# lbcb-sci/raven

Measured on NVIDIA H100. Metric: overlaps/s, higher is better.
Workload: dtype u64

## Files before the change

### raven_b200/csrc/map.cu

```cuda
#include <algorithm>

#include "engine.cuh"
#include "seed.cuh"

namespace rvn {

namespace {

constexpr int kThreads = 256;

__global__ void __launch_bounds__(kThreads)
ProbeKernel(IndexView ix, ValView q_val,
            const uint64_t* __restrict__ q_org, uint64_t q_begin, uint64_t n_q,
            bool avoid_equal, bool avoid_symmetric,
            uint32_t* __restrict__ cnt, uint32_t* __restrict__ first,
            uint8_t* __restrict__ filt) {
  const uint64_t i = static_cast<uint64_t>(blockIdx.x) * kThreads + threadIdx.x;
  if (i >= n_q) return;
  const uint32_t lhs_id = static_cast<uint32_t>(q_org[q_begin + i] >> 32);
  ProbeRun(ix, q_val[q_begin + i], lhs_id, avoid_equal, avoid_symmetric, first + i, cnt + i,
           filt + i);
}

struct HitStore {
// ... 431 lines not shown
      const uint64_t* Pb = P + jb;
      const IdxT* idx = MINI + jb + b;
      const bool strand = G[jb] & 1;
      for (uint32_t kk = 1, l = 0; kk <= longest; ++kk) {
        const uint32_t prev = static_cast<uint32_t>(Pb[idx[kk - 1]] >> 32);
        const uint32_t cur =
            kk < longest ? static_cast<uint32_t>(Pb[idx[kk]] >> 32) : 0xFFFFFFFFu;
        if (cur - prev > cp.gap) {
          if (kk - l >= cp.chain) {
            uint32_t lm = 0, lb_ = 0, le = 0, rm = 0, rb_ = 0, re = 0;
            for (uint32_t m = l; m < kk; ++m) {
              const uint64_t pp = Pb[idx[m]];
              const uint32_t lp = static_cast<uint32_t>(pp >> 32);
              if (lp > le) {
                lm += le - lb_;
                lb_ = lp;
              }
              le = lp + cp.k;
              uint32_t rp = static_cast<uint32_t>(pp);
              rp = strand ? rp : (1U << 31) - (rp + cp.k - 1);
              if (rp > re) {
                rm += re - rb_;
                rb_ = rp;
              }
              re = rp + cp.k;
            }
            lm += le - lb_;
            rm += re - rb_;
            if (min(lm, rm) >= cp.matches) ++emitted;
          }
          l = kk;
        }
      }
    }
    wk.CNT[b] = emitted;
    wk.IE[b] = static_cast<IdxT>(longest);
  }
  __syncthreads();

  uint32_t carry = 0;
  __shared__ uint32_t sh_total;
  {
    uint32_t local = 0;
    for (uint32_t b = threadIdx.x; b < nb; b += THREADS) local += wk.CNT[b];
    uint32_t tot;
    BlockExclusiveSum<uint32_t, THREADS>(local, sm32, &tot);
    if (threadIdx.x == 0) {
      sh_total = tot;
      sh_base = tot ? atomicAdd(ovl_counter, static_cast<unsigned long long>(tot))
                    : 0ULL;
    }
    __syncthreads();
  }
  const uint32_t total = sh_total;
  const uint64_t base = sh_base;
  *out_base = base;
  if (total == 0 || base + total > ovl_cap) return total;

  for (uint32_t b0 = 0; b0 < nb; b0 += THREADS) {
    const uint32_t b = b0 + threadIdx.x;
    const uint32_t mine = b < nb ? wk.CNT[b] : 0;
    uint32_t tot;
    const uint32_t ex = BlockExclusiveSum<uint32_t, THREADS>(mine, sm32, &tot);
    if (mine) {
      rvn_overlap* dst = ovl_raw + base + carry + ex;
      uint64_t* kdst = ovl_key ? ovl_key + base + carry + ex : nullptr;
      uint32_t seq = carry + ex;
      const uint32_t jb = wk.IB[b];
      const uint32_t longest = wk.IE[b];
      const uint64_t* Pb = P + jb;
      const IdxT* idx = MINI + jb + b;
      const bool strand = G[jb] & 1;
      const uint32_t rhs_id = static_cast<uint32_t>(G[jb] & 0xFFFFFFFFu) >> 1;
      for (uint32_t kk = 1, l = 0; kk <= longest; ++kk) {
        const uint32_t prev = static_cast<uint32_t>(Pb[idx[kk - 1]] >> 32);
        const uint32_t cur =
            kk < longest ? static_cast<uint32_t>(Pb[idx[kk]] >> 32) : 0xFFFFFFFFu;
        if (cur - prev > cp.gap) {
          if (kk - l >= cp.chain) {
            uint32_t lm = 0, lb_ = 0, le = 0, rm = 0, rb_ = 0, re = 0;
            for (uint32_t m = l; m < kk; ++m) {
              const uint64_t pp = Pb[idx[m]];
              const uint32_t lp = static_cast<uint32_t>(pp >> 32);
              if (lp > le) {
                lm += le - lb_;
                lb_ = lp;
              }
              le = lp + cp.k;
              uint32_t rp = static_cast<uint32_t>(pp);
              rp = strand ? rp : (1U << 31) - (rp + cp.k - 1);
              if (rp > re) {
                rm += re - rb_;
                rb_ = rp;
              }
              re = rp + cp.k;
            }
            lm += le - lb_;
            rm += re - rb_;
            if (min(lm, rm) >= cp.matches) {
              const uint64_t pf = Pb[idx[l]], pl = Pb[idx[kk - 1]];
              rvn_overlap o;
              o.lhs_id = lhs_id;
              o.lhs_begin = static_cast<uint32_t>(pf >> 32);
              o.lhs_end = cp.k + static_cast<uint32_t>(pl >> 32);
              o.rhs_id = rhs_id;
              o.rhs_begin = strand ? static_cast<uint32_t>(pf)
                                   : static_cast<uint32_t>(pl);
              o.rhs_end = cp.k + (strand ? static_cast<uint32_t>(pl)
                                         : static_cast<uint32_t>(pf));
              o.score = min(lm, rm);
              o.strand = strand;
              *dst++ = o;
              if (kdst) *kdst++ = key_hi | seq++;
            }
          }
          l = kk;
        }
      }
    }
    carry += tot;
  }
  return total;
}

constexpr uint32_t kChainSmemCap = 65535;
constexpr uint32_t kSplitMaxTable = 8192;
constexpr uint32_t kPairMaxHits = 8191;
constexpr uint32_t kThreadPairMax = 48;

struct GroupDesc {
  uint32_t hit_off, cnt, gid, lhs_id;
};

struct SplitLayout {
  uint32_t hs, gpad;
  size_t hk, hc, gl, bytes;
};

__host__ __device__ inline SplitLayout MakeSplitLayout(uint32_t n) {
  SplitLayout L;
  uint32_t hs = 64;
  while (hs < n + 1 && hs < kSplitMaxTable) hs <<= 1;
  L.hs = hs;
  uint32_t gpad = 2;
  while (gpad < n / 4 + 1 && gpad < hs) gpad <<= 1;
  L.gpad = gpad;
  size_t o = 0;
  L.hk = o; o += 4ULL * hs;
  L.hc = o; o += 4ULL * hs;
  L.gl = o; o += 8ULL * gpad;
  L.bytes = (o + 15) & ~size_t(15);
  return L;
}

__device__ __forceinline__ uint32_t HashGid(uint32_t x) {
  x ^= x >> 16;
  x *= 0x7feb352dU;
  x ^= x >> 15;
  x *= 0x846ca68bU;
  x ^= x >> 16;
  return x;
}

template <int THREADS, int MINB>
__global__ void __launch_bounds__(THREADS, MINB)
SplitKernel(const uint64_t* __restrict__ h_grp, const uint64_t* __restrict__ h_pos,
            const uint64_t* __restrict__ read_hit_off,
            const uint32_t* __restrict__ lhs_ids,
            const uint32_t* __restrict__ read_list,
            unsigned long long* __restrict__ totals,
            GroupDesc* __restrict__ desc, uint32_t* __restrict__ desc_cnt,
            uint32_t* __restrict__ desc_idx, uint32_t* __restrict__ g_diag,
            uint64_t* __restrict__ g_pos, uint64_t* __restrict__ group_loc,
            uint32_t* __restrict__ fallback_list,
            unsigned int* __restrict__ fallback_cnt) {
  extern __shared__ __align__(16) unsigned char smem[];
  __shared__ uint32_t sm32[34];
  __shared__ uint32_t sh_bail;
  __shared__ unsigned long long sh_gbase, sh_hbase;
  const uint32_t r = read_list[blockIdx.x];
  const uint64_t hb = read_hit_off[r];
  const uint32_t n = static_cast<uint32_t>(read_hit_off[r + 1] - hb);
  const SplitLayout L = MakeSplitLayout(n);
  uint32_t* HK = reinterpret_cast<uint32_t*>(smem + L.hk);
  uint32_t* HC = reinterpret_cast<uint32_t*>(smem + L.hc);
  uint64_t* GL = reinterpret_cast<uint64_t*>(smem + L.gl);
  const uint32_t hmask = L.hs - 1;
  const uint64_t* hg = h_grp + hb;
  const uint64_t* hp = h_pos + hb;

  for (uint32_t i = threadIdx.x; i < L.hs; i += THREADS) {
    HK[i] = 0xFFFFFFFFu;
    HC[i] = 0;
  }
  if (threadIdx.x == 0) sh_bail = 0;
  __syncthreads();
  for (uint32_t i = threadIdx.x; i < n; i += THREADS) {
    const uint32_t gid = static_cast<uint32_t>(hg[i] >> 32);
    uint32_t s = HashGid(gid) & hmask;
    uint32_t probes = 0;
    while (true) {
      const uint32_t prev = atomicCAS(&HK[s], 0xFFFFFFFFu, gid);
      if (prev == 0xFFFFFFFFu || prev == gid) break;
      s = (s + 1) & hmask;
      if (++probes > hmask) {
        sh_bail = 1;
        break;
      }
    }
    if (probes <= hmask) atomicAdd(&HC[s], 1u);
  }
  __syncthreads();
  if (sh_bail) {
    if (threadIdx.x == 0) fallback_list[atomicAdd(fallback_cnt, 1u)] = r;
    return;
  }

  uint32_t carry = 0;
  for (uint32_t b = 0; b < L.hs; b += THREADS) {
    const uint32_t s = b + threadIdx.x;
    const uint32_t cnt = s < L.hs ? HC[s] : 0;
    const uint32_t keep = cnt >= 4;
    if (cnt > kPairMaxHits) sh_bail = 1;
    uint32_t tot;
    const uint32_t ex = BlockExclusiveSum<uint32_t, THREADS>(
        keep ? ((cnt << 16) | 1u) : 0u, sm32, &tot);
    if (s < L.hs) {
      if (keep) {
        const uint32_t at = carry + ex;
        GL[at & 0xFFFF] = (static_cast<uint64_t>(HK[s]) << 32) | s;
        HC[s] = (cnt << 16) | (at >> 16);
      } else {
        HC[s] = 0xFFFFFFFFu;
      }
    }
    carry += tot;
  }
  const uint32_t ng = carry & 0xFFFF, nh = carry >> 16;
  __syncthreads();
  if (sh_bail) {
    if (threadIdx.x == 0) fallback_list[atomicAdd(fallback_cnt, 1u)] = r;
    return;
  }
  if (ng == 0) {
    if (threadIdx.x == 0) group_loc[r] = 0;
    return;
  }

  uint32_t gpad = 2;
  while (gpad < ng) gpad <<= 1;
  for (uint32_t i = ng + threadIdx.x; i < gpad; i += THREADS) GL[i] = ~0ULL;
  if (threadIdx.x == 0) {
    sh_gbase = atomicAdd(&totals[0], static_cast<unsigned long long>(ng));
    sh_hbase = atomicAdd(&totals[1], static_cast<unsigned long long>(nh));
  }
  __syncthreads();
  for (uint32_t size = 2; size <= gpad; size <<= 1) {
    for (uint32_t stride = size >> 1; stride > 0; stride >>= 1) {
      for (uint32_t t = threadIdx.x; t < (gpad >> 1); t += THREADS) {
        const uint32_t i = 2 * t - (t & (stride - 1));
        const uint32_t j = i + stride;
        const uint64_t a = GL[i], c2 = GL[j];
        if ((a > c2) == ((i & size) == 0)) {
          GL[i] = c2;
          GL[j] = a;
        }
      }
      __syncthreads();
    }
  }
  const uint64_t gbase = sh_gbase, hbase = sh_hbase;
  const uint32_t lhs_id = lhs_ids[r];
  for (uint32_t q = threadIdx.x; q < ng; q += THREADS) {
    const uint64_t e = GL[q];
    const uint32_t s = static_cast<uint32_t>(e);
    const uint32_t v = HC[s];
    GroupDesc d;
    d.hit_off = static_cast<uint32_t>(hbase) + (v & 0xFFFF);
    d.cnt = v >> 16;
    d.gid = static_cast<uint32_t>(e >> 32);
    d.lhs_id = lhs_id;
    desc[gbase + q] = d;
    desc_cnt[gbase + q] = d.cnt;
    desc_idx[gbase + q] = static_cast<uint32_t>(gbase + q);
    HC[s] = v & 0xFFFF;
  }
  if (threadIdx.x == 0) group_loc[r] = (gbase << 24) | ng;
  __syncthreads();

  for (uint32_t i = threadIdx.x; i < n; i += THREADS) {
    const uint64_t g = hg[i];
    const uint32_t gid = static_cast<uint32_t>(g >> 32);
    uint32_t s = HashGid(gid) & hmask;
    while (HK[s] != gid) s = (s + 1) & hmask;
    if (HC[s] == 0xFFFFFFFFu) continue;
    const uint64_t at = hbase + atomicAdd(&HC[s], 1u);
    g_diag[at] = static_cast<uint32_t>(g);
    g_pos[at] = hp[i];
  }
}

struct Column {
  uint64_t* P;
  uint32_t* D;
  uint32_t T;
  __device__ __forceinline__ uint64_t& p(uint32_t i) const { return P[i * T]; }
  __device__ __forceinline__ uint32_t& d(uint32_t i) const { return D[i * T]; }
};

__device__ __forceinline__ void BandChain(const Column& c, uint32_t jb, uint32_t ie,
                                          bool strand, uint32_t lhs_id,
                                          uint32_t rhs_id, const ChainParams& cp,
                                          uint64_t key_hi, uint32_t* seq,
                                          rvn_overlap* __restrict__ out,
                                          uint64_t* __restrict__ out_key,
                                          unsigned long long* __restrict__ out_cnt,
                                          uint64_t out_cap) {
  const uint32_t len = ie - jb;
  if (len < cp.chain) return;
  for (uint32_t a = 1; a < len; ++a) {
    const uint64_t pv = c.p(jb + a);
    if (c.p(jb + a - 1) <= pv) continue;
    uint32_t lo = 0, hi = a - 1;
    while (lo < hi) {
      const uint32_t mid = (lo + hi) >> 1;
      if (c.p(jb + mid) > pv) {
        hi = mid;
      } else {
        lo = mid + 1;
      }
    }
    for (uint32_t b = a; b > lo; --b) c.p(jb + b) = c.p(jb + b - 1);
    c.p(jb + lo) = pv;
  }
  auto mini_get = [&](uint32_t x) -> uint32_t { return c.d(jb + x) & 0xFFFFu; };
  auto mini_set = [&](uint32_t x, uint32_t v) {
    c.d(jb + x) = (c.d(jb + x) & 0xFFFF0000u) | v;
  };
  auto pred_get = [&](uint32_t x) -> uint32_t { return c.d(jb + x) >> 16; };
  auto pred_set = [&](uint32_t x, uint32_t v) {
    c.d(jb + x) = (c.d(jb + x) & 0xFFFFu) | (v << 16);
  };
  uint32_t longest = 0;
  for (uint32_t t = 0; t < len; ++t) {
    const uint64_t cur = c.p(jb + t);
    const uint32_t cl = static_cast<uint32_t>(cur >> 32);
    const uint32_t cr = static_cast<uint32_t>(cur);
    uint32_t lo = 1, hi = longest;
    while (lo <= hi) {
      const uint32_t mid = lo + (hi - lo) / 2;
      const uint64_t tail = c.p(jb + mini_get(mid - 1));
      const uint32_t tl = static_cast<uint32_t>(tail >> 32);
      const uint32_t tr = static_cast<uint32_t>(tail);
      if (tl < cl && (strand ? tr < cr : tr > cr)) {
        lo = mid + 1;
      } else {
        hi = mid - 1;
      }
    }
    pred_set(t, lo > 1 ? mini_get(lo - 2) : 0u);
    mini_set(lo - 1, t);
    longest = max(longest, lo);
  }
  if (longest < cp.chain) return;
  {
    uint32_t j = mini_get(longest - 1);
    for (uint32_t i = 0; i < longest; ++i) {
      const uint32_t pj = pred_get(j);
      mini_set(longest - 1 - i, j);
      j = pj;
    }
  }
  for (uint32_t kk = 1, l = 0; kk <= longest; ++kk) {
    const uint32_t prev = static_cast<uint32_t>(c.p(jb + mini_get(kk - 1)) >> 32);
    const uint32_t cur = kk < longest
                             ? static_cast<uint32_t>(c.p(jb + mini_get(kk)) >> 32)
                             : 0xFFFFFFFFu;
    if (cur - prev > cp.gap) {
      if (kk - l >= cp.chain) {
        uint32_t lm = 0, lb_ = 0, le = 0, rm = 0, rb_ = 0, re = 0;
        for (uint32_t m = l; m < kk; ++m) {
          const uint64_t pp = c.p(jb + mini_get(m));
          const uint32_t lp = static_cast<uint32_t>(pp >> 32);
          if (lp > le) {
            lm += le - lb_;
            lb_ = lp;
          }
          le = lp + cp.k;
          uint32_t rp = static_cast<uint32_t>(pp);
          rp = strand ? rp : (1U << 31) - (rp + cp.k - 1);
          if (rp > re) {
            rm += re - rb_;
            rb_ = rp;
          }
          re = rp + cp.k;
        }
        lm += le - lb_;
        rm += re - rb_;
        if (min(lm, rm) >= cp.matches) {
          const uint64_t pf = c.p(jb + mini_get(l)), pl = c.p(jb + mini_get(kk - 1));
          rvn_overlap o;
          o.lhs_id = lhs_id;
          o.lhs_begin = static_cast<uint32_t>(pf >> 32);
          o.lhs_end = cp.k + static_cast<uint32_t>(pl >> 32);
          o.rhs_id = rhs_id;
          o.rhs_begin = strand ? static_cast<uint32_t>(pf) : static_cast<uint32_t>(pl);
          o.rhs_end = cp.k + (strand ? static_cast<uint32_t>(pl)
                                     : static_cast<uint32_t>(pf));
          o.score = min(lm, rm);
          o.strand = strand;
          const unsigned long long slot = atomicAdd(out_cnt, 1ULL);
          if (slot < out_cap) {
            out[slot] = o;
            out_key[slot] = key_hi | (*seq)++;
          }
        }
      }
      l = kk;
    }
  }
}

__global__ void GroupChainKernel(const GroupDesc* __restrict__ desc,
                                 const uint32_t* __restrict__ order, uint64_t first,
                                 uint64_t last, uint32_t m_cap,
                                 const uint32_t* __restrict__ g_diag,
                                 const uint64_t* __restrict__ g_pos, ChainParams cp,
                                 rvn_overlap* __restrict__ out,
                                 uint64_t* __restrict__ out_key,
                                 unsigned long long* __restrict__ out_cnt,
                                 uint64_t out_cap) {
  extern __shared__ __align__(16) unsigned char smem[];
  const uint32_t T = blockDim.x;
  const uint64_t t = first + static_cast<uint64_t>(blockIdx.x) * T + threadIdx.x;
  if (t >= last) return;
  Column c;
  c.P = reinterpret_cast<uint64_t*>(smem) + threadIdx.x;
  c.D = reinterpret_cast<uint32_t*>(smem + 8ULL * m_cap * T) + threadIdx.x;
  c.T = T;
  const uint32_t g = order[t];
  const GroupDesc d = desc[g];
  const uint32_t m = d.cnt;
  for (uint32_t i = 0; i < m; ++i) {
    c.p(i) = g_pos[d.hit_off + i];
    c.d(i) = g_diag[d.hit_off + i];
  }
  for (uint32_t a = 1; a < m; ++a) {
    const uint32_t dv = c.d(a);
    const uint64_t pv = c.p(a);
    uint32_t lo = 0, hi = a;
    while (lo < hi) {
      const uint32_t mid = (lo + hi) >> 1;
      const uint32_t dm = c.d(mid);
      if (dm > dv || (dm == dv && c.p(mid) > pv)) {
        hi = mid;
      } else {
        lo = mid + 1;
      }
    }
    for (uint32_t b = a; b > lo; --b) {
      c.d(b) = c.d(b - 1);
      c.p(b) = c.p(b - 1);
    }
    c.d(lo) = dv;
    c.p(lo) = pv;
  }
  const bool strand = d.gid & 1;
  const uint32_t rhs_id = d.gid >> 1;
  const uint64_t key_hi = static_cast<uint64_t>(g) << 16;
  uint32_t seq = 0;
  bool open = false;
  uint32_t ob = 0, oe = 0;
  for (uint32_t i = 1, j = 0; i <= m; ++i) {
    if (i == m || c.d(i) - c.d(j) > cp.bandwidth) {
      if (i - j >= 4) {
        if (open && oe > j) {
          oe = i;
        } else {
          if (open) {
            BandChain(c, ob, oe, strand, d.lhs_id, rhs_id, cp, key_hi, &seq, out,
                      out_key, out_cnt, out_cap);
          }
          ob = j;
          oe = i;
          open = true;
        }
      }
      ++j;
      while (j < i && (i == m || c.d(i) - c.d(j) > cp.bandwidth)) ++j;
    }
  }
  if (open) {
    BandChain(c, ob, oe, strand, d.lhs_id, rhs_id, cp, key_hi, &seq, out, out_key,
              out_cnt, out_cap);
  }
}

constexpr int kPairThreads = 64;

__host__ __device__ inline size_t PairChainSmem(uint32_t npad) {
  const uint32_t n = npad - 1, nb = n / 4 + 1;
  size_t o = 16ULL * npad;
  o += 2ULL * (n + nb + 2) + 2ULL * (n + 1) + 2ULL * 2 * nb;
  o = (o + 3) & ~size_t(3);
  o += 4ULL * nb;
  return (o + 15) & ~size_t(15);
}

__global__ void __launch_bounds__(kPairThreads)
PairChainKernel(const GroupDesc* __restrict__ desc, const uint32_t* __restrict__ order,
                uint64_t first, uint32_t npad, const uint32_t* __restrict__ g_diag,
                const uint64_t* __restrict__ g_pos, ChainParams cp,
                rvn_overlap* __restrict__ out, uint64_t* __restrict__ out_key,
                unsigned long long* __restrict__ out_cnt, uint64_t out_cap) {
  extern __shared__ __align__(16) unsigned char smem[];
  __shared__ uint32_t sm32[34];
  const uint32_t g = order[first + blockIdx.x];
  const GroupDesc d = desc[g];
  const uint32_t n = d.cnt;
  const uint32_t ncap = npad - 1, nbmax = ncap / 4 + 1;
  ChainWork<uint16_t> wk;
  wk.G = reinterpret_cast<uint64_t*>(smem);
  wk.P = wk.G + npad;
  wk.LB = reinterpret_cast<uint16_t*>(wk.P + npad);
  wk.PD = wk.LB + (ncap + nbmax + 2);
  wk.IB = wk.PD + (ncap + 1);
  wk.IE = wk.IB + nbmax;
  wk.CNT = reinterpret_cast<uint32_t*>(
      (reinterpret_cast<uintptr_t>(wk.IE + nbmax) + 3) & ~uintptr_t(3));
  uint32_t np2 = 8;
  while (np2 < n + 1) np2 <<= 1;
  for (uint32_t i = threadIdx.x; i < np2; i += kPairThreads) {
    wk.G[i] = i < n ? (static_cast<uint64_t>(d.gid) << 32) | g_diag[d.hit_off + i] : ~0ULL;
    wk.P[i] = i < n ? g_pos[d.hit_off + i] : ~0ULL;
  }
  __syncthreads();
  uint64_t base = 0;
  ChainRead<uint16_t, kPairThreads>(wk, n, np2, d.lhs_id, cp, sm32, out, out_cnt, out_cap, &base,
                                    out_key, static_cast<uint64_t>(g) << 16);
}

__global__ void SizeClassStarts(const uint32_t* __restrict__ sorted_cnt, uint64_t n,
                                const uint32_t* __restrict__ bound, uint32_t n_bounds,
                                uint64_t* __restrict__ start) {
  const uint32_t i = threadIdx.x;
  if (i >= n_bounds) return;
  const uint32_t bnd = bound[i];
  uint64_t lo = 0, hi = n;
  while (lo < hi) {
    const uint64_t mid = lo + (hi - lo) / 2;
    if (sorted_cnt[mid] > bnd) {
      lo = mid + 1;
    } else {
      hi = mid;
    }
  }
  start[i] = lo;
}

__global__ void IotaU32(uint32_t* __restrict__ out, uint64_t n) {
  const uint64_t i = static_cast<uint64_t>(blockIdx.x) * blockDim.x + threadIdx.x;
  if (i < n) out[i] = static_cast<uint32_t>(i);
}

__global__ void GatherOverlapsByIndex(const rvn_overlap* __restrict__ src,
                                      const uint32_t* __restrict__ idx, uint64_t n,
                                      rvn_overlap* __restrict__ dst) {
  const uint64_t i = static_cast<uint64_t>(blockIdx.x) * blockDim.x + threadIdx.x;
  if (i >= n * 2) return;
  const uint4* s = reinterpret_cast<const uint4*>(src);
  reinterpret_cast<uint4*>(dst)[i] = s[static_cast<uint64_t>(idx[i >> 1]) * 2 + (i & 1)];
}

__global__ void LocateReadOverlaps(const uint64_t* __restrict__ sorted_key,
                                   uint64_t n_keys,
                                   const uint32_t* __restrict__ read_list,
                                   uint32_t n_list,
                                   const uint64_t* __restrict__ group_loc,
                                   uint64_t base0, uint64_t* __restrict__ ovl_loc) {
  const uint32_t i = blockIdx.x * blockDim.x + threadIdx.x;
  if (i >= n_list) return;
  const uint32_t r = read_list[i];
  const uint64_t gl = group_loc[r];
  const uint64_t gbase = gl >> 24, ng = gl & 0xFFFFFF;
  if (ng == 0) {
    ovl_loc[r] = 0;
    return;
  }
  auto lower = [&](uint64_t key) {
    uint64_t lo = 0, hi = n_keys;
    while (lo < hi) {
      const uint64_t mid = lo + (hi - lo) / 2;
      if (sorted_key[mid] < key) {
        lo = mid + 1;
      } else {
        hi = mid;
      }
    }
    return lo;
  };
  const uint64_t a = lower(gbase << 16), b = lower((gbase + ng) << 16);
  ovl_loc[r] = b > a ? ((base0 + a) << 24) | (b - a) : 0;
}

__global__ void __launch_bounds__(kThreads)
ChainKernelGlobal(const uint64_t* __restrict__ h_grp,
                  const uint64_t* __restrict__ h_pos,
                  const uint64_t* __restrict__ read_hit_off,
                  const uint32_t* __restrict__ lhs_ids,
                  const uint32_t* __restrict__ big_reads,
                  const uint64_t* __restrict__ slab64_off,
                  const uint64_t* __restrict__ slab32_off,
                  uint64_t* __restrict__ slab64, uint32_t* __restrict__ slab32,
                  ChainParams cp, rvn_overlap* __restrict__ ovl_raw,
                  unsigned long long* __restrict__ ovl_counter,
                  uint64_t ovl_cap, uint64_t* __restrict__ ovl_loc) {
  __shared__ uint32_t sm32[34];
  const uint32_t r = big_reads[blockIdx.x];
  const uint64_t hb = read_hit_off[r];
  const uint32_t n = static_cast<uint32_t>(read_hit_off[r + 1] - hb);
  uint32_t npad = 8;
  while (npad < n + 1) npad <<= 1;

  ChainWork<uint32_t> wk;
  wk.G = slab64 + slab64_off[blockIdx.x];
  wk.P = wk.G + npad;
  const uint32_t nbmax = n / 4 + 1;
  wk.LB = slab32 + slab32_off[blockIdx.x];
  wk.PD = wk.LB + (n + nbmax + 2);
  wk.IB = wk.PD + (n + 1);
  wk.IE = wk.IB + nbmax;
  wk.CNT = wk.IE + nbmax;

  for (uint32_t i = threadIdx.x; i < npad; i += kThreads) {
    wk.G[i] = i < n ? h_grp[hb + i] : ~0ULL;
    wk.P[i] = i < n ? h_pos[hb + i] : ~0ULL;
  }
  __syncthreads();
  uint64_t base = 0;
  const uint32_t total = ChainRead<uint32_t, kThreads>(
      wk, n, npad, lhs_ids[r], cp, sm32, ovl_raw, ovl_counter, ovl_cap,
      &base);
  if (threadIdx.x == 0) ovl_loc[r] = total ? (base << 24) | total : 0;
}

__global__ void OverlapCounts(const uint64_t* __restrict__ ovl_loc, uint64_t n,
                              uint32_t* __restrict__ cnt) {
  const uint64_t i = static_cast<uint64_t>(blockIdx.x) * blockDim.x + threadIdx.x;
  if (i < n) cnt[i] = static_cast<uint32_t>(ovl_loc[i] & 0xFFFFFF);
}

__global__ void ReorderOverlaps(const rvn_overlap* __restrict__ raw,
                                const uint64_t* __restrict__ ovl_loc,
                                const uint64_t* __restrict__ ovl_off,
                                uint32_t n_reads, rvn_overlap* __restrict__ out) {
  const uint32_t r = blockIdx.x * (blockDim.x / 32) + (threadIdx.x >> 5);
  if (r >= n_reads) return;
  const uint64_t loc = ovl_loc[r];
  const uint32_t cnt = static_cast<uint32_t>(loc & 0xFFFFFF);
  const uint64_t src = loc >> 24, dst = ovl_off[r];
  const uint4* s = reinterpret_cast<const uint4*>(raw + src);
  uint4* d = reinterpret_cast<uint4*>(out + dst);
  for (uint32_t i = threadIdx.x & 31; i < cnt * 2; i += 32) d[i] = s[i];
}

void JoinSweep(Ctx& c, uint32_t first) {
  const uint32_t nr = c.i_last - first;
  const uint64_t t0 = first - c.qt_first, base = c.h_q_off[t0];
  c.h_j_off.resize(nr + 1ULL);
  for (uint32_t i = 0; i <= nr; ++i) c.h_j_off[i] = c.h_q_off[t0 + i] - base;
  const uint64_t n_q = c.h_j_off[nr];
  uint64_t* off = c.j_off.reserve(nr + 1ULL);
  RVN_CUDA(cudaMemcpyAsync(off, c.h_j_off.data(), (nr + 1ULL) * sizeof(uint64_t),
                           cudaMemcpyHostToDevice, c.stream));
  uint32_t* cursor = c.j_cursor.reserve(nr + 1ULL);
  uint64_t* packed = c.j_packed.reserve(n_q + 1);
  RVN_CUDA(cudaMemsetAsync(cursor, 0, (nr + 1ULL) * sizeof(uint32_t), c.stream));
  RVN_CUDA(cudaMemsetAsync(packed, 0, (n_q + 1) * sizeof(uint64_t), c.stream));
  if (c.i_n > 0 && n_q > 0) {
    JoinView jv{ValView{c.i_val.get(), c.i_is32 ? 1 : 0}, c.i_org.get(), c.i_n, c.occurrence,
                c.qt_val.get() + t0, c.qt_pos.get() + t0, first, c.i_last};
    JoinSweepKernel<<<CeilDiv(c.i_n, kThreads), kThreads, 0, c.stream>>>(jv, off, cursor,
                                                                          packed);
    RVN_LAUNCH_CHECK();
    ++c.launches;
  }
  RVN_CUDA(cudaStreamSynchronize(c.stream));
  c.j_gen = c.i_gen;
  c.j_occurrence = c.occurrence;
  c.j_first = first;
}

struct HitCounts {
  uint64_t n_q = 0, n_hits = 0;
};

void ReadHitRanges(Ctx& c, const uint64_t* hit_off, const uint64_t* read_off, uint64_t q_begin,
                   uint32_t nr, uint64_t* read_hit_off, std::vector<uint64_t>& h_rho) {
  GatherU64<<<CeilDiv(nr + 1ULL, kThreads), kThreads, 0, c.stream>>>(
      hit_off, read_off, q_begin, nr + 1ULL, read_hit_off);
  RVN_LAUNCH_CHECK();
  ++c.launches;
  RVN_CUDA(cudaMemcpyAsync(h_rho.data(), read_hit_off, (nr + 1ULL) * sizeof(uint64_t),
                           cudaMemcpyDeviceToHost, c.stream));
  RVN_CUDA(cudaStreamSynchronize(c.stream));
}

HitCounts JoinHits(Ctx& c, uint32_t first, uint32_t last, uint64_t* read_hit_off,
                   std::vector<uint64_t>& h_rho) {
  const uint32_t nr = last - first;
  HitCounts h;
  const bool sweep = c.j_gen != c.i_gen || c.j_occurrence != c.occurrence || first < c.j_first;
  if (sweep && !(c.qt_valid && c.qt_first <= first && c.i_last <= c.qt_last)) {
    EnsureThresholds(c, first, c.i_last);
  }
  TimerBegin(c, "probe");
  if (sweep) JoinSweep(c, first);
  const uint64_t b0 = first - c.j_first;
  const uint64_t q_begin = c.h_j_off[b0];
  h.n_q = c.h_j_off[b0 + nr] - q_begin;
  const uint64_t* packed = c.j_packed.get() + q_begin;
  uint64_t* hit_off = c.m_hit_off.reserve(h.n_q + 2);
  if (h.n_q > 0) {
    uint32_t* cnt = c.m_cnt.reserve(h.n_q + 1);
    UnpackJoin<<<CeilDiv(h.n_q, kThreads), kThreads, 0, c.stream>>>(packed, h.n_q, cnt);
    RVN_LAUNCH_CHECK();
    ++c.launches;
    ExclusiveScanU32(c, cnt, hit_off, h.n_q);
    h.n_hits = ReadU64(c, hit_off + h.n_q);
  } else {
    RVN_CUDA(cudaMemsetAsync(hit_off, 0, sizeof(uint64_t), c.stream));
  }
  TimerEnd(c);
  TimerBegin(c, "expand");
  uint64_t* hg = c.h_grp.reserve(h.n_hits + 1);
  uint64_t* hp = c.h_pos.reserve(h.n_hits + 1);
  if (h.n_hits > 0) {
    ExpandJoinKernel<<<CeilDiv(h.n_q, kThreads), kThreads, 0, c.stream>>>(
        c.i_org.get(), packed, h.n_q, hit_off, hg, hp);
    RVN_LAUNCH_CHECK();
    ++c.launches;
  }
  ReadHitRanges(c, hit_off, c.j_off.get() + b0, q_begin, nr, read_hit_off, h_rho);
  TimerEnd(c);
  c.r_filt_off.reserve(nr + 2ULL);
  for (uint32_t i = 0; i <= nr; ++i) c.r_filt_off.get()[i] = 0;
  return h;
}

void FilteredPositions(Ctx& c, const uint8_t* filt, const uint64_t* qo, uint64_t q_begin,
                       uint64_t n_q, const uint64_t* read_off, uint32_t nr) {
  uint32_t* f32 = c.m_first.get();
  FilteredFlagsToU32<<<CeilDiv(n_q, kThreads), kThreads, 0, c.stream>>>(
      filt, n_q, f32);
  uint64_t* fpos = c.m_filt_off.reserve(n_q + 2);
  ExclusiveScanU32(c, f32, fpos, n_q);
  const uint64_t n_filtered = ReadU64(c, fpos + n_q);
  uint32_t* fout = c.m_filtered.reserve(n_filtered + 1);
  ScatterFiltered<<<CeilDiv(n_q, kThreads), kThreads, 0, c.stream>>>(
      filt, fpos, qo, q_begin, n_q, fout);
  RVN_LAUNCH_CHECK();
  c.launches += 2;
  uint64_t* froff = c.m_ovl_off.reserve(nr + 2ULL);
  GatherU64<<<CeilDiv(nr + 1ULL, kThreads), kThreads, 0, c.stream>>>(
      fpos, read_off, q_begin, nr + 1ULL, froff);
  RVN_LAUNCH_CHECK();
  ++c.launches;
  uint32_t* hf = c.r_filtered.reserve(n_filtered + 1);
  RVN_CUDA(cudaMemcpyAsync(hf, fout, n_filtered * sizeof(uint32_t),
                           cudaMemcpyDeviceToHost, c.stream));
  RVN_CUDA(cudaMemcpyAsync(c.r_filt_off.get(), froff,
                           (nr + 1ULL) * sizeof(uint64_t),
                           cudaMemcpyDeviceToHost, c.stream));
  RVN_CUDA(cudaStreamSynchronize(c.stream));
}

HitCounts ProbeHits(Ctx& c, uint32_t first, uint32_t last, bool avoid_equal,
                    bool avoid_symmetric, bool minhash, bool want_filtered,
                    uint64_t* read_hit_off, std::vector<uint64_t>& h_rho) {
  const uint32_t nr = last - first;
  HitCounts h;
  const uint64_t *qo, *d_read_off;
  ValView qv;
  const std::vector<uint64_t>* h_read_off;
  uint64_t off_base_read;
  if (minhash) {
    if (!(c.q_valid && c.q_first <= first && last <= c.q_last)) {
      EnsureMicromizers(c, first, last);
    }
    qv = ValView{c.q_val.get(), c.q_is32 ? 1 : 0};
    qo = c.q_org.get();
    d_read_off = c.q_off.get();
    h_read_off = &c.h_q_off;
    off_base_read = first - c.q_first;
  } else {
    if (!(c.s_valid && c.s_first <= first && last <= c.s_last)) {
      EnsureSketch(c, first, last);
    }
    qv = ValView{c.s_val.get(), c.s_is32 ? 1 : 0};
    qo = c.s_org.get();
    d_read_off = c.s_off.get();
    h_read_off = &c.h_s_off;
    off_base_read = first - c.s_first;
  }
  const uint64_t q_begin = (*h_read_off)[off_base_read];
  const uint64_t n_q = (*h_read_off)[off_base_read + nr] - q_begin;
  h.n_q = n_q;

  IndexView ix{ValView{c.i_val.get(), c.i_is32 ? 1 : 0}, c.i_org.get(), c.i_bucket.get(), c.i_n,
               c.i_shift, c.occurrence, c.i_limit};

  TimerBegin(c, "probe");
  uint32_t* cnt = c.m_cnt.reserve(n_q + 1);
  uint32_t* frst = c.m_first.reserve(n_q + 1);
  uint8_t* filt = c.m_filt.reserve(n_q + 1);
  uint64_t* hit_off = c.m_hit_off.reserve(n_q + 2);
  const bool suffix = (avoid_equal && avoid_symmetric && c.i_sorted_ids) ||
                      (!avoid_equal && !avoid_symmetric);
  if (n_q > 0) {
    if (suffix && n_q >= (1u << 16) && n_q < 0xFFFFFFFFULL) {
      uint64_t* k1 = c.m_sq_key.reserve(n_q + 2);
      uint64_t* k2 = c.m_sq_key2.reserve(n_q);
      uint32_t* v1 = c.m_sq_idx.reserve(n_q);
      uint32_t* v2 = c.m_sq_idx2.reserve(n_q);
      IotaU32<<<CeilDiv(n_q, kThreads), kThreads, 0, c.stream>>>(v1, n_q);
      const int hi_bit = static_cast<int>(2 * c.prm.k);
      int w_q;
      ValView sorted_qv;
      if (qv.is32) {
        const uint32_t* src = static_cast<const uint32_t*>(qv.p) + q_begin;
        uint32_t* a32 = reinterpret_cast<uint32_t*>(k1);
        uint32_t* b32 = a32 + n_q + (n_q & 1);
        w_q = RadixSortPairs(c, src, a32, b32, v1, v2, v1, n_q, 0, hi_bit);
        sorted_qv = ValView{w_q < 0 ? src : (w_q == 0 ? a32 : b32), 1};
      } else {
        const uint64_t* src = static_cast<const uint64_t*>(qv.p) + q_begin;
        w_q = RadixSortPairs(c, src, k1, k2, v1, v2, v1, n_q, 0, hi_bit);
        sorted_qv = ValView{w_q < 0 ? src : (w_q == 0 ? k1 : k2), 0};
      }
      const uint32_t* sorted_qi = w_q == 0 ? v2 : v1;
      uint64_t* packed = (qv.is32 || w_q == 0) ? k2 : k1;
      ProbeSortedKernel<<<CeilDiv(n_q, kThreads), kThreads, 0, c.stream>>>(
          ix, sorted_qv, sorted_qi, qo, q_begin, n_q, avoid_equal, packed);
      UnpackProbe<<<CeilDiv(n_q, kThreads), kThreads, 0, c.stream>>>(packed, n_q, cnt, frst, filt);
      c.launches += (2 * c.prm.k + 7) / 8 + 5;
    } else if (suffix) {
      ProbeSuffixKernel<<<CeilDiv(n_q, kThreads), kThreads, 0, c.stream>>>(
          ix, qv, qo, q_begin, n_q, avoid_equal, cnt, frst, filt);
    } else {
      ProbeKernel<<<CeilDiv(n_q, kThreads), kThreads, 0, c.stream>>>(
          ix, qv, qo, q_begin, n_q, avoid_equal, avoid_symmetric, cnt, frst, filt);
    }
    RVN_LAUNCH_CHECK();
    ++c.launches;
    ExclusiveScanU32(c, cnt, hit_off, n_q);
    h.n_hits = ReadU64(c, hit_off + n_q);
  } else {
    RVN_CUDA(cudaMemsetAsync(hit_off, 0, sizeof(uint64_t), c.stream));
  }
  TimerEnd(c);
  TimerBegin(c, "expand");
  uint64_t* hg = c.h_grp.reserve(h.n_hits + 1);
  uint64_t* hp = c.h_pos.reserve(h.n_hits + 1);
  if (h.n_hits > 0) {
    if (suffix) {
      ExpandWarpKernel<<<CeilDiv(n_q, kThreads), kThreads, 0, c.stream>>>(
          ix, qo, q_begin, n_q, cnt, frst, hit_off, hg, hp);
    } else {
      ExpandKernel<<<CeilDiv(n_q, kThreads), kThreads, 0, c.stream>>>(
          ix, qv, qo, q_begin, n_q, avoid_equal, avoid_symmetric, cnt, frst,
          hit_off, hg, hp);
    }
    RVN_LAUNCH_CHECK();
    ++c.launches;
  }
  ReadHitRanges(c, hit_off, d_read_off + off_base_read, q_begin, nr, read_hit_off, h_rho);
  TimerEnd(c);

  c.r_filt_off.reserve(nr + 2ULL);
  for (uint32_t i = 0; i <= nr; ++i) c.r_filt_off.get()[i] = 0;
  if (want_filtered && n_q > 0) {
    FilteredPositions(c, filt, qo, q_begin, n_q, d_read_off + off_base_read, nr);
  }
  return h;
}

}

uint64_t ChainGroupedHits(Ctx& c, const uint64_t* hg, const uint64_t* hp,
                          const uint64_t* read_hit_off,
                          const std::vector<uint64_t>& h_rho, const uint32_t* lhs_ids,
                          uint32_t nr, uint64_t n_hits, uint64_t n_q) {
  TimerBegin(c, "chain");
  ChainParams cp{c.prm.k, c.prm.bandwidth, c.prm.chain, c.prm.matches, c.prm.gap};
  const uint64_t ovl_cap = n_hits / std::max(1u, std::min(c.prm.chain, 4u)) + 16;
  rvn_overlap* raw = c.m_ovl_raw.reserve(ovl_cap);
  uint64_t* loc = c.m_ovl_loc.reserve(nr + 1ULL);
  uint64_t* counter = c.m_counter.reserve((1u << 16) + 8);
  RVN_CUDA(cudaMemsetAsync(counter, 0, sizeof(uint64_t), c.stream));
  RVN_CUDA(cudaMemsetAsync(loc, 0, (nr + 1ULL) * sizeof(uint64_t), c.stream));

  static const uint32_t kBounds[] = {256, 512, 1024, 2048, 4096, 8192, 65536};
  constexpr int kClasses = sizeof(kBounds) / sizeof(kBounds[0]);
  std::vector<uint32_t> cls[kClasses];
  std::vector<uint32_t> big;
  const bool fast_ok = c.prm.chain >= 1;
  for (uint32_t i = 0; i < nr; ++i) {
    const uint64_t n = h_rho[i + 1] - h_rho[i];
    if (n < 4) continue;
    if (n > kChainSmemCap || !fast_ok) {
      big.push_back(i);
      continue;
    }
    int k = 0;
    while (kBounds[k] < n + 1) ++k;
    cls[k].push_back(i);
  }
  uint64_t n_fast_ovl = 0;
  {
    size_t total = 0;
    for (auto& v : cls) total += v.size();
    uint32_t* d_list = c.m_first.reserve(std::max<size_t>(total, n_q) + 1);
    uint32_t* d_fb = c.m_fallback.reserve(nr + 4ULL);
    RVN_CUDA(cudaMemsetAsync(d_fb, 0, 2 * sizeof(uint32_t), c.stream));
    std::vector<uint32_t> flat;
    flat.reserve(total);
    for (int k = kClasses - 1; k >= 0; --k) {
      flat.insert(flat.end(), cls[k].begin(), cls[k].end());
    }
    if (total) {
      RVN_CUDA(cudaMemcpyAsync(d_list, flat.data(), total * sizeof(uint32_t),
                               cudaMemcpyHostToDevice, c.stream));
      RVN_CUDA(cudaStreamSynchronize(c.stream));

      const uint64_t max_groups = n_hits / 4 + 1;
      GroupDesc* desc = reinterpret_cast<GroupDesc*>(
          c.m_desc.reserve(max_groups * (sizeof(GroupDesc) / 4)));
      uint32_t* dcnt = c.m_desc_cnt.reserve(max_groups);
      uint32_t* didx = c.m_desc_idx.reserve(max_groups);
      uint32_t* dcnt2 = c.m_desc_cnt2.reserve(max_groups);
      uint32_t* didx2 = c.m_desc_idx2.reserve(max_groups);
      uint32_t* g_diag = c.m_gdiag.reserve(n_hits + 1);
      uint64_t* g_pos = c.m_gpos.reserve(n_hits + 1);
      uint64_t* group_loc = c.m_group_loc.reserve(nr + 1ULL);
      RVN_CUDA(cudaMemsetAsync(counter, 0, 4 * sizeof(uint64_t), c.stream));
      auto* ctr = reinterpret_cast<unsigned long long*>(counter);

      size_t off = 0;
      for (int k = kClasses - 1; k >= 0; --k) {
        const unsigned cnt = static_cast<unsigned>(cls[k].size());
        if (cnt == 0) continue;
        const size_t smem = MakeSplitLayout(kBounds[k] - 1).bytes;
        const uint32_t* lst = d_list + off;
        off += cnt;
        if (kBounds[k] > 2048) {
          auto kern = SplitKernel<256, 2>;
          RVN_CUDA(cudaFuncSetAttribute(
              kern, cudaFuncAttributeMaxDynamicSharedMemorySize,
              static_cast<int>(MakeSplitLayout(kChainSmemCap).bytes)));
          kern<<<cnt, 256, smem, c.stream>>>(hg, hp, read_hit_off, lhs_ids, lst,
                                             ctr + 1, desc, dcnt, didx, g_diag, g_pos,
                                             group_loc, d_fb + 2, d_fb);
        } else {
          auto kern = SplitKernel<128, 8>;
          kern<<<cnt, 128, smem, c.stream>>>(hg, hp, read_hit_off, lhs_ids, lst,
                                             ctr + 1, desc, dcnt, didx, g_diag, g_pos,
                                             group_loc, d_fb + 2, d_fb);
        }
        RVN_LAUNCH_CHECK();
        ++c.launches;
      }
      uint64_t* hpin = c.pin64.reserve(8);
      RVN_CUDA(cudaMemcpyAsync(hpin, counter, 4 * sizeof(uint64_t),
                               cudaMemcpyDeviceToHost, c.stream));
      std::vector<uint32_t> fb(2);
      RVN_CUDA(cudaMemcpyAsync(fb.data(), d_fb, 2 * sizeof(uint32_t),
                               cudaMemcpyDeviceToHost, c.stream));
      RVN_CUDA(cudaStreamSynchronize(c.stream));
      const uint64_t n_groups = hpin[1];
      const uint32_t nfb = fb[0];
      if (nfb) {
        fb.resize(nfb);
        RVN_CUDA(cudaMemcpyAsync(fb.data(), d_fb + 2, nfb * sizeof(uint32_t),
                                 cudaMemcpyDeviceToHost, c.stream));
        RVN_CUDA(cudaStreamSynchronize(c.stream));
        std::sort(fb.begin(), fb.end());
        big.insert(big.end(), fb.begin(), fb.end());
      }
      if (n_groups >= 0xFFFFFFFFULL) throw LimitError("2^32 or more seed pairs");
      if (hpin[2] >= 0xFFFFFFFFULL) throw LimitError("2^32 or more chained seed hits in one flush");

      if (n_groups) {
        const int w_desc = RadixSortPairs(c, dcnt, dcnt2, dcnt, didx, didx2, didx, n_groups, 0, 13,
                                          true);
        const uint32_t* sorted_cnt = w_desc == 0 ? dcnt2 : dcnt;
        const uint32_t* sorted_idx = w_desc == 0 ? didx2 : didx;
        rvn_overlap* tmp_ovl = c.m_ovl_tmp.reserve(ovl_cap);
        uint64_t* key = c.m_okey.reserve(ovl_cap);
        uint64_t* key2 = c.m_okey2.reserve(ovl_cap);
        uint32_t* oidx = c.m_oidx.reserve(ovl_cap);
        uint32_t* oidx2 = c.m_oidx2.reserve(ovl_cap);
        static const uint32_t kGB[] = {8191, 4095, 2047, 1023, 511, 255, 127, 63,
                                       kThreadPairMax, 32, 24, 16, 8};
        constexpr uint32_t kNB = sizeof(kGB) / sizeof(kGB[0]);
        constexpr uint32_t kFirstThreadClass = 8;
        uint32_t* d_bounds = c.m_bounds.reserve(kNB);
        uint64_t* d_starts = c.m_starts.reserve(kNB + 1);
        RVN_CUDA(cudaMemcpyAsync(d_bounds, kGB, sizeof(kGB), cudaMemcpyHostToDevice,
                                 c.stream));
        SizeClassStarts<<<1, 32, 0, c.stream>>>(sorted_cnt, n_groups, d_bounds, kNB, d_starts);
        uint64_t h_starts[kNB + 1];
        RVN_CUDA(cudaMemcpyAsync(h_starts, d_starts, kNB * sizeof(uint64_t),
                                 cudaMemcpyDeviceToHost, c.stream));
        RVN_CUDA(cudaStreamSynchronize(c.stream));
        h_starts[kNB] = n_groups;
        h_starts[0] = 0;
        RVN_CUDA(cudaFuncSetAttribute(GroupChainKernel,
                                      cudaFuncAttributeMaxDynamicSharedMemorySize,
                                      200 * 1024));
        RVN_CUDA(cudaFuncSetAttribute(PairChainKernel,
                                      cudaFuncAttributeMaxDynamicSharedMemorySize,
                                      static_cast<int>(PairChainSmem(8192))));
        for (uint32_t b = 0; b < kNB; ++b) {
          const uint64_t lo = h_starts[b], hi = h_starts[b + 1];
          if (hi <= lo) continue;
          if (b < kFirstThreadClass) {
            const uint32_t npad = kGB[b] + 1;
            PairChainKernel<<<static_cast<unsigned>(hi - lo), kPairThreads, PairChainSmem(npad),
                              c.stream>>>(desc, sorted_idx, lo, npad, g_diag, g_pos, cp, tmp_ovl,
                                          key, ctr + 3, ovl_cap);
          } else {
            uint32_t threads = 128;
            while (threads > 8 && 12ULL * kGB[b] * threads > 196 * 1024) threads >>= 1;
            const size_t smem = 12ULL * kGB[b] * threads;
            GroupChainKernel<<<CeilDiv(hi - lo, threads), threads, smem, c.stream>>>(
                desc, sorted_idx, lo, hi, kGB[b], g_diag, g_pos, cp, tmp_ovl, key, ctr + 3,
                ovl_cap);
          }
          RVN_LAUNCH_CHECK();
          ++c.launches;
        }
        n_fast_ovl = ReadU64(c, counter + 3);
        if (n_fast_ovl > ovl_cap) throw LimitError("overlap slab overflow");
        if (n_fast_ovl >= 0xFFFFFFFFULL) throw LimitError("2^32 or more overlaps");
        if (n_fast_ovl) {
          IotaU32<<<CeilDiv(n_fast_ovl, kThreads), kThreads, 0, c.stream>>>(
              oidx, n_fast_ovl);
          int key_bits = 17;
          while (key_bits < 64 && (1ULL << (key_bits - 16)) < n_groups) ++key_bits;
          const int w_ovl = RadixSortPairs(c, key, key2, key, oidx, oidx2, oidx, n_fast_ovl, 0,
                                           key_bits);
          const uint64_t* sorted_key = w_ovl == 0 ? key2 : key;
          const uint32_t* sorted_oidx = w_ovl == 0 ? oidx2 : oidx;
          GatherOverlapsByIndex<<<CeilDiv(n_fast_ovl * 2, kThreads), kThreads, 0,
                                  c.stream>>>(tmp_ovl, sorted_oidx, n_fast_ovl, raw);
          LocateReadOverlaps<<<CeilDiv(total, kThreads), kThreads, 0, c.stream>>>(
              sorted_key, n_fast_ovl, d_list, static_cast<uint32_t>(total),
              group_loc, 0, loc);
          RVN_LAUNCH_CHECK();
          c.launches += 3;
        }
      }
      RVN_CUDA(cudaMemcpyAsync(counter, &n_fast_ovl, sizeof(uint64_t),
                               cudaMemcpyHostToDevice, c.stream));
      RVN_CUDA(cudaStreamSynchronize(c.stream));
    }
  }
  if (!big.empty()) {
    std::vector<uint64_t> off64(big.size() + 1, 0), off32(big.size() + 1, 0);
    for (size_t i = 0; i < big.size(); ++i) {
      const uint64_t n = h_rho[big[i] + 1] - h_rho[big[i]];
      if (n >= 0x7FFFFFFFULL) throw LimitError("a query has 2^31 or more hits");
      uint64_t npad = 8;
      while (npad < n + 1) npad <<= 1;
      const uint64_t nbmax = n / 4 + 1;
      off64[i + 1] = off64[i] + 2 * npad;
      off32[i + 1] = off32[i] + (n + nbmax + 2) + (n + 1) + 3 * nbmax + 4;
    }
    uint64_t* slab64 = c.m_scratch64.reserve(off64.back() + 2 * (big.size() + 1) + 8);
    uint32_t* slab32 = c.m_scratch32.reserve(off32.back() + big.size() + 8);
    uint64_t* d_off64 = slab64 + off64.back();
    uint64_t* d_off32 = d_off64 + big.size() + 1;
    uint32_t* d_big = slab32 + off32.back();
    RVN_CUDA(cudaMemcpyAsync(d_off64, off64.data(), (big.size() + 1) * 8,
                             cudaMemcpyHostToDevice, c.stream));
    RVN_CUDA(cudaMemcpyAsync(d_off32, off32.data(), (big.size() + 1) * 8,
                             cudaMemcpyHostToDevice, c.stream));
    RVN_CUDA(cudaMemcpyAsync(d_big, big.data(), big.size() * 4,
                             cudaMemcpyHostToDevice, c.stream));
    ChainKernelGlobal<<<static_cast<unsigned>(big.size()), kThreads, 0,
                        c.stream>>>(
        hg, hp, read_hit_off, lhs_ids, d_big, d_off64, d_off32, slab64, slab32, cp,
        raw, reinterpret_cast<unsigned long long*>(counter), ovl_cap, loc);
    RVN_LAUNCH_CHECK();
    ++c.launches;
    RVN_CUDA(cudaStreamSynchronize(c.stream));
  }

  uint32_t* ocnt = c.m_cnt.reserve(nr + 1ULL);
  uint64_t* ooff = c.m_ovl_off.reserve(nr + 2ULL);
  uint64_t n_ovl = 0;
  if (nr > 0) {
    OverlapCounts<<<CeilDiv(nr, kThreads), kThreads, 0, c.stream>>>(loc, nr, ocnt);
    RVN_LAUNCH_CHECK();
    ++c.launches;
    ExclusiveScanU32(c, ocnt, ooff, nr);
    n_ovl = ReadU64(c, ooff + nr);
  } else {
    RVN_CUDA(cudaMemsetAsync(ooff, 0, sizeof(uint64_t), c.stream));
  }
  if (n_ovl > ovl_cap) throw LimitError("overlap slab overflow");
  rvn_overlap* ordered = c.m_ovl.reserve(n_ovl + 1);
  if (n_ovl > 0) {
    ReorderOverlaps<<<CeilDiv(nr, kThreads / 32), kThreads, 0, c.stream>>>(
        raw, loc, ooff, nr, ordered);
    RVN_LAUNCH_CHECK();
    ++c.launches;
  }
  TimerEnd(c);
  return n_ovl;
}

void MapRange(Ctx& c, uint32_t first, uint32_t last, bool avoid_equal,
              bool avoid_symmetric, bool minhash, bool want_filtered,
              bool fetch) {
  if (!c.i_valid) throw StateError("Map before Minimize");
  c.r_valid = false;
  const uint32_t nr = last - first;

  const bool join = c.self_join && minhash && avoid_equal && avoid_symmetric && !want_filtered &&
                    c.i_from_sketch && c.i_sorted_ids && c.ids_identity && first >= c.i_first &&
                    last <= c.i_last;
  uint64_t* read_hit_off = c.m_read_hit_off.reserve(nr + 2ULL);
  std::vector<uint64_t> h_rho(nr + 1ULL);
  const HitCounts h =
      join ? JoinHits(c, first, last, read_hit_off, h_rho)
           : ProbeHits(c, first, last, avoid_equal, avoid_symmetric, minhash, want_filtered,
                       read_hit_off, h_rho);
  const uint64_t n_q = h.n_q, n_hits = h.n_hits;
  const uint64_t* hg = c.h_grp.get();
  const uint64_t* hp = c.h_pos.get();

  if (c.keep_hits) {
    uint64_t* g = c.r_hit_grp.reserve(n_hits + 1);
    uint64_t* p = c.r_hit_pos.reserve(n_hits + 1);
    uint64_t* o = c.r_hit_off.reserve(nr + 2ULL);
    RVN_CUDA(cudaMemcpyAsync(g, hg, n_hits * sizeof(uint64_t),
                             cudaMemcpyDeviceToHost, c.stream));
    RVN_CUDA(cudaMemcpyAsync(p, hp, n_hits * sizeof(uint64_t),
                             cudaMemcpyDeviceToHost, c.stream));
    for (uint32_t i = 0; i <= nr; ++i) o[i] = h_rho[i];
    RVN_CUDA(cudaStreamSynchronize(c.stream));
    c.r_n_hits = n_hits;
  }

  const uint64_t n_ovl =
      ChainGroupedHits(c, hg, hp, read_hit_off, h_rho, c.d_ids.get() + first, nr, n_hits, n_q);
  const rvn_overlap* ordered = c.m_ovl.get();
  const uint64_t* ooff = c.m_ovl_off.get();

  if (fetch) {
    rvn_overlap* ho = c.r_ovl.reserve(n_ovl + 1);
    uint64_t* hoff = c.r_ovl_off.reserve(nr + 2ULL);
    RVN_CUDA(cudaMemcpyAsync(ho, ordered, n_ovl * sizeof(rvn_overlap),
                             cudaMemcpyDeviceToHost, c.stream));
    RVN_CUDA(cudaMemcpyAsync(hoff, ooff, (nr + 1ULL) * sizeof(uint64_t),
                             cudaMemcpyDeviceToHost, c.stream));
    RVN_CUDA(cudaStreamSynchronize(c.stream));
  }
  c.r_n_ovl = n_ovl;
  c.m_hits = n_hits;
  c.m_first_read = first;
  c.m_last_read = last;
  c.r_valid = fetch;

  uint64_t qbases = 0;
  for (uint32_t r = first; r < last; ++r) qbases += c.h_len[r];
  c.stats.query_bases += qbases;
  c.stats.query_records += n_q;
  c.stats.hits += n_hits;
  c.stats.overlaps += n_ovl;
}

}
```

Baseline: 56.77 million.

## Pack diagonal and lhs position into one 64-bit sort key in GroupChainKernel

GroupChainKernel now stores each hit as a single 64-bit key of diagonal in the high word and lhs position in the low word, in place of separate position and diagonal arrays. The insertion sort compares single u64 values and skips elements already in order, and BandChain rebuilds lhs/rhs positions from the key for each band. The per-hit bookkeeping shrinks to 16 bits with 8-bit mini and pred fields, cutting shared memory from 12 to 10 bytes per hit, and the block size is fixed at 64 threads. The 8-bit fields cap chain indices at 255, which could be a correctness risk for larger groups, and the reconstructed rhs depends on the diagonal encoding being exact.

```diff
diff --git a/profiles/chain_split.py b/profiles/chain_split.py
--- /dev/null
+++ b/profiles/chain_split.py
@@ -0,0 +1,127 @@
+from __future__ import annotations
+
+import argparse
+import json
+import os
+import subprocess
+import sys
+
+ROOT = os.path.dirname(os.path.dirname(os.path.abspath(__file__)))
+sys.path.insert(0, ROOT)
+
+SEED = 20260924
+K, W, FREQ, KMAX = 15, 5, 0.001, 32
+READS, GENOME, MEAN_LEN = 200_000, 50_000_000, 10_000
+
+OPEN = ("SplitKernel", "ChainKernelGlobal")
+CLOSE = "ReorderOverlaps"
+
+
+def card():
+    try:
+        out = subprocess.run(["nvidia-smi", "--query-gpu=name,power.limit,clocks.max.sm",
+                              "--format=csv,noheader"], capture_output=True, text=True,
+                             timeout=30).stdout.strip().splitlines()
+        return out[0] if out else "unknown"
+    except (OSError, subprocess.SubprocessError):
+        return "unknown"
+
+
+def short_name(name):
+    s = name.replace("(anonymous namespace)::", "").replace("void ", "").replace("rvn::", "")
+    s = s.replace("unsigned long long", "u64").replace("unsigned long", "u64")
+    s = s.replace("unsigned int", "u32")
+    return s.split("(")[0]
+
+
+def algorithmic_bytes(short, st):
+    nh, no = st["hits"], st["overlaps"]
+    if short.startswith("SplitKernel"):
+        return 16 * nh
+    if short.startswith("GatherOverlapsByIndex") or short.startswith("ReorderOverlaps"):
+        return 64 * no
+    return None
+
+
+def main():
+    ap = argparse.ArgumentParser()
+    ap.add_argument("--steps", type=int, default=3)
+    ap.add_argument("--warmup", type=int, default=2)
+    ap.add_argument("--reads", type=int, default=READS)
+    ap.add_argument("--out", default=None, metavar="DIR",
+                    help="also write the tables as DIR/chain_split.json")
+    a = ap.parse_args()
+
+    import torch
+    from torch.profiler import ProfilerActivity, profile
+
+    if not torch.cuda.is_available():
+        raise SystemExit("chain_split.py needs a CUDA device")
+    from bench import synth
+    from raven_b200 import engine
+
+    rs = synth.make_reads(SEED, GENOME, a.reads, MEAN_LEN)
+    stream = torch.cuda.current_stream()
+    eng = engine.Engine(device=0, stream=stream.cuda_stream)
+    eng.configure(K, W)
+    eng.upload(rs)
+
+    def step():
+        eng.find_overlaps_and_create_piles(FREQ, KMAX, False, 0, fetch=False)
+
+    dev = card()
+    print(f"card: {dev}")
+    for _ in range(a.warmup):
+        step()
+    torch.cuda.synchronize()
+    eng.set_option("reset_stats", 1)
+    with profile(activities=[ProfilerActivity.CUDA]) as prof:
+        for _ in range(a.steps):
+            step()
+        torch.cuda.synchronize()
+    phases = eng.timings()
+    st = eng.stats()
+
+    evs = sorted((e for e in prof.events() if e.device_type == torch.autograd.DeviceType.CUDA),
+                 key=lambda e: e.time_range.start)
+    per = {}
+    inside = False
+    for e in evs:
+        if any(k in e.name for k in OPEN):
+            inside = True
+        if not inside or "Memcpy" in e.name or "Memset" in e.name:
+            continue
+        d = per.setdefault(short_name(e.name), [0.0, 0])
+        d[0] += (e.time_range.end - e.time_range.start) / 1e3
+        d[1] += 1
+        if CLOSE in e.name:
+            inside = False
+    rows = []
+    for name, (ms, cnt) in sorted(per.items(), key=lambda x: -x[1][0]):
+        ms_step, launches = ms / a.steps, cnt / a.steps
+        b = algorithmic_bytes(name, st)
+        rate = (b / (ms_step * 1e-3) / 1e12) if b and ms_step > 0 else None
+        rows.append({"kernel": name, "ms_per_step": round(ms_step, 3),
+                     "launches_per_step": launches,
+                     "gbytes": None if b is None else round(b / 1e9, 3),
+                     "tb_per_s": None if rate is None else round(rate, 3)})
+    total = sum(r["ms_per_step"] for r in rows)
+    print(f"\nC2 stage 1, {a.reads} reads: {a.steps} steps; per step {st['hits']} hits, "
+          f"{st['overlaps']} overlaps")
+    print(f"  phase chain (last step, engine timer): {phases.get('chain', 0):.2f} ms; "
+          f"kernels of the chain window: {total:.2f} ms per step")
+    print(f"  {'kernel':<58} {'ms/step':>8} {'launch':>6} {'GB':>7} {'TB/s':>6}")
+    for r in rows:
+        print(f"  {r['kernel'][:58]:<58} {r['ms_per_step']:8.3f} {r['launches_per_step']:6.1f} "
+              f"{'' if r['gbytes'] is None else r['gbytes']:>7} "
+              f"{'' if r['tb_per_s'] is None else r['tb_per_s']:>6}")
+    if a.out:
+        os.makedirs(a.out, exist_ok=True)
+        with open(os.path.join(a.out, "chain_split.json"), "w") as f:
+            json.dump({"card": dev, "reads": a.reads, "steps": a.steps, "phases_ms": phases,
+                       "stats": st, "kernels": rows}, f, indent=1)
+    eng.close()
+
+
+if __name__ == "__main__":
+    main()
diff --git a/raven_b200/csrc/map.cu b/raven_b200/csrc/map.cu
--- a/raven_b200/csrc/map.cu
+++ b/raven_b200/csrc/map.cu
@@ -757,11 +757,24 @@
 
 struct Column {
   uint64_t* P;
-  uint32_t* D;
+  uint16_t* M;
   uint32_t T;
   __device__ __forceinline__ uint64_t& p(uint32_t i) const { return P[i * T]; }
-  __device__ __forceinline__ uint32_t& d(uint32_t i) const { return D[i * T]; }
+  __device__ __forceinline__ uint16_t& m(uint32_t i) const { return M[i * T]; }
+  __device__ __forceinline__ uint32_t d(uint32_t i) const {
+    return static_cast<uint32_t>(P[i * T] >> 32);
+  }
 };
+
+__device__ __forceinline__ uint64_t HitKey(uint32_t diag, uint64_t pos) {
+  return (static_cast<uint64_t>(diag) << 32) | (pos >> 32);
+}
+
+__device__ __forceinline__ uint64_t HitPositions(uint64_t key, bool strand) {
+  const uint32_t diag = static_cast<uint32_t>(key >> 32), lhs = static_cast<uint32_t>(key);
+  const uint32_t rhs = strand ? diag + lhs - (3u << 30) : diag - lhs;
+  return (static_cast<uint64_t>(lhs) << 32) | rhs;
+}
 
 __device__ __forceinline__ void BandChain(const Column& c, uint32_t jb, uint32_t ie,
                                           bool strand, uint32_t lhs_id,
@@ -773,6 +786,7 @@
                                           uint64_t out_cap) {
   const uint32_t len = ie - jb;
   if (len < cp.chain) return;
+  for (uint32_t x = jb; x < ie; ++x) c.p(x) = HitPositions(c.p(x), strand);
   for (uint32_t a = 1; a < len; ++a) {
     const uint64_t pv = c.p(jb + a);
     if (c.p(jb + a - 1) <= pv) continue;
@@ -788,13 +802,13 @@
     for (uint32_t b = a; b > lo; --b) c.p(jb + b) = c.p(jb + b - 1);
     c.p(jb + lo) = pv;
   }
-  auto mini_get = [&](uint32_t x) -> uint32_t { return c.d(jb + x) & 0xFFFFu; };
+  auto mini_get = [&](uint32_t x) -> uint32_t { return c.m(jb + x) & 0xFFu; };
   auto mini_set = [&](uint32_t x, uint32_t v) {
-    c.d(jb + x) = (c.d(jb + x) & 0xFFFF0000u) | v;
+    c.m(jb + x) = static_cast<uint16_t>((c.m(jb + x) & 0xFF00u) | v);
   };
-  auto pred_get = [&](uint32_t x) -> uint32_t { return c.d(jb + x) >> 16; };
+  auto pred_get = [&](uint32_t x) -> uint32_t { return c.m(jb + x) >> 8; };
   auto pred_set = [&](uint32_t x, uint32_t v) {
-    c.d(jb + x) = (c.d(jb + x) & 0xFFFFu) | (v << 16);
+    c.m(jb + x) = static_cast<uint16_t>((c.m(jb + x) & 0xFFu) | (v << 8));
   };
   uint32_t longest = 0;
   for (uint32_t t = 0; t < len; ++t) {
@@ -891,34 +905,26 @@
   if (t >= last) return;
   Column c;
   c.P = reinterpret_cast<uint64_t*>(smem) + threadIdx.x;
-  c.D = reinterpret_cast<uint32_t*>(smem + 8ULL * m_cap * T) + threadIdx.x;
+  c.M = reinterpret_cast<uint16_t*>(smem + 8ULL * m_cap * T) + threadIdx.x;
   c.T = T;
   const uint32_t g = order[t];
   const GroupDesc d = desc[g];
   const uint32_t m = d.cnt;
-  for (uint32_t i = 0; i < m; ++i) {
-    c.p(i) = g_pos[d.hit_off + i];
-    c.d(i) = g_diag[d.hit_off + i];
-  }
+  for (uint32_t i = 0; i < m; ++i) c.p(i) = HitKey(g_diag[d.hit_off + i], g_pos[d.hit_off + i]);
   for (uint32_t a = 1; a < m; ++a) {
-    const uint32_t dv = c.d(a);
-    const uint64_t pv = c.p(a);
-    uint32_t lo = 0, hi = a;
+    const uint64_t kv = c.p(a);
+    if (c.p(a - 1) <= kv) continue;
+    uint32_t lo = 0, hi = a - 1;
     while (lo < hi) {
       const uint32_t mid = (lo + hi) >> 1;
-      const uint32_t dm = c.d(mid);
-      if (dm > dv || (dm == dv && c.p(mid) > pv)) {
+      if (c.p(mid) > kv) {
         hi = mid;
       } else {
         lo = mid + 1;
       }
     }
-    for (uint32_t b = a; b > lo; --b) {
-      c.d(b) = c.d(b - 1);
-      c.p(b) = c.p(b - 1);
-    }
-    c.d(lo) = dv;
-    c.p(lo) = pv;
+    for (uint32_t b = a; b > lo; --b) c.p(b) = c.p(b - 1);
+    c.p(lo) = kv;
   }
   const bool strand = d.gid & 1;
   const uint32_t rhs_id = d.gid >> 1;
@@ -1485,9 +1491,8 @@
                               c.stream>>>(desc, sorted_idx, lo, npad, g_diag, g_pos, cp, tmp_ovl,
                                           key, ctr + 3, ovl_cap);
           } else {
-            uint32_t threads = 128;
-            while (threads > 8 && 12ULL * kGB[b] * threads > 196 * 1024) threads >>= 1;
-            const size_t smem = 12ULL * kGB[b] * threads;
+            constexpr uint32_t threads = 64;
+            const size_t smem = 10ULL * kGB[b] * threads;
             GroupChainKernel<<<CeilDiv(hi - lo, threads), threads, smem, c.stream>>>(
                 desc, sorted_idx, lo, hi, kGB[b], g_diag, g_pos, cp, tmp_ovl, key, ctr + 3,
                 ovl_cap);
```

After: 57.35 million (median of 6 runs). +1.0%, better.
